# dschleef/schroedinger

Hardware: AMD Instinct MI355X
Metric: Mpix/s IIWT+OBMC decode, 2160p s16 (higher is better)
Workload: dtype s16

## Files before the change

### include/schro_hip.h

```cpp
#ifndef SCHRO_HIP_H
#define SCHRO_HIP_H

#include <stddef.h>
#include <stdint.h>

#ifdef __cplusplus
extern "C" {
#endif

#define SCHRO_HIP_OK 0
#define SCHRO_HIP_EINVAL (-1)
#define SCHRO_HIP_EDEVICE (-2)
#define SCHRO_HIP_ENOMEM (-3)
#define SCHRO_HIP_EUNSUPPORTED (-4)
#define SCHRO_HIP_ESKIPPED (-5)
#define SCHRO_HIP_ENEEDS_RESIDUAL (-6)

#define SCHRO_EXEC_DOMAIN_HIP 0x0004
#define SCHRO_MEMORY_DOMAIN_HIP 0x0008

#define SCHRO_HIP_FORMAT_DEPTH(f) ((f) & 0xc)
#define SCHRO_HIP_FORMAT_DEPTH_U8 0x00
#define SCHRO_HIP_FORMAT_DEPTH_S16 0x04
#define SCHRO_HIP_FORMAT_DEPTH_S32 0x08
// ... 19 lines not shown
int schro_hip_upload_2d (SchroHipContext * ctx, void *dst, int dst_stride,
    const void *src, int src_stride, int row_bytes, int height);
int schro_hip_download_2d (SchroHipContext * ctx, void *dst, int dst_stride,
    const void *src, int src_stride, int row_bytes, int height);
int schro_hip_memset (SchroHipContext * ctx, void *dst, int value,
    size_t bytes);
void *schro_hip_host_alloc (size_t size);
void schro_hip_host_free (void *ptr);
int schro_hip_upload_2d_async (SchroHipContext * ctx, void *dst, int dst_stride,
    const void *src, int src_stride, int row_bytes, int height);
int schro_hip_download_2d_async (SchroHipContext * ctx, void *dst, int dst_stride,
    const void *src, int src_stride, int row_bytes, int height);
int schro_hip_queue_synchronize (SchroHipContext * ctx, int queue);
int schro_hip_queue_set_cu_mask (SchroHipContext * ctx, int queue, const uint32_t * mask, int words);
int schro_hip_synchronize (SchroHipContext * ctx);
void *schro_hip_stream (SchroHipContext * ctx);

#define SCHRO_HIP_QUEUES 4
#define SCHRO_HIP_QUEUE_H2D 2
#define SCHRO_HIP_QUEUE_D2H 3
int schro_hip_context_select_queue (SchroHipContext * ctx, int queue);
int schro_hip_context_queue (SchroHipContext * ctx);
int schro_hip_queue_wait (SchroHipContext * ctx, int waiter, int signaller);
#define SCHRO_HIP_MARKS 16
int schro_hip_queue_mark (SchroHipContext * ctx, int mark);
int schro_hip_queue_wait_mark (SchroHipContext * ctx, int mark);
int schro_hip_queue_mark_synchronize (SchroHipContext * ctx, int mark);

int schro_hip_timer_begin (SchroHipContext * ctx);
float schro_hip_timer_end (SchroHipContext * ctx);

#define SCHRO_HIP_KERNEL_IIWT_FINEST 0
#define SCHRO_HIP_KERNEL_IIWT_COARSE 1
#define SCHRO_HIP_KERNEL_UPSAMPLE 2
#define SCHRO_HIP_KERNEL_OBMC 3
#define SCHRO_HIP_KERNEL_CONVERT 4
#define SCHRO_HIP_KERNEL_SLICES 5
#define SCHRO_HIP_KERNEL_DC_PREDICT 6
#define SCHRO_HIP_KERNEL_DEQUANT 7
#define SCHRO_HIP_KERNEL_QUANTISE 8
#define SCHRO_HIP_KERNEL_QUANTISE_DC 9
#define SCHRO_HIP_KERNEL_CLASSES 10
int schro_hip_profile_enable (SchroHipContext * ctx, int enable);
int schro_hip_profile_reset (SchroHipContext * ctx);
int schro_hip_profile_read (SchroHipContext * ctx, int kernel_class,
    double *total_ms, int *launches);

#define SCHRO_HIP_OBMC_ROUTE_ROW 0
#define SCHRO_HIP_OBMC_ROUTE_ITEM 1
#define SCHRO_HIP_OBMC_ROUTE_GENERAL 2
#define SCHRO_HIP_OBMC_ROUTE_STRIP 3
#define SCHRO_HIP_OBMC_ROUTES 4
int schro_hip_obmc_routes (SchroHipContext * ctx, long long counts[SCHRO_HIP_OBMC_ROUTES], int reset);

#define SCHRO_HIP_V210_ROUTE_HAAR3 0
#define SCHRO_HIP_V210_ROUTE_LEVEL 1
#define SCHRO_HIP_V210_ROUTE_TWO_PASS 2
#define SCHRO_HIP_V210_ROUTES 3
int schro_hip_v210_routes (SchroHipContext * ctx, long long counts[SCHRO_HIP_V210_ROUTES], int reset);

#define SCHRO_HIP_PACK8_ROUTE_LEVEL 0
#define SCHRO_HIP_PACK8_ROUTE_TWO_PASS 1
#define SCHRO_HIP_PACK8_ROUTES 2
int schro_hip_pack8_routes (SchroHipContext * ctx, long long counts[SCHRO_HIP_PACK8_ROUTES], int reset);

#define SCHRO_HIP_WIDE_ROUTE_LEVEL 0
#define SCHRO_HIP_WIDE_ROUTE_TWO_PASS 1
#define SCHRO_HIP_WIDE_ROUTES 2
int schro_hip_wide_routes (SchroHipContext * ctx, long long counts[SCHRO_HIP_WIDE_ROUTES], int reset);


typedef struct {
  const void *src;
  int src_stride;
  void *dst;
  int dst_stride;
  int width;
  int height;
  const uint8_t *pred;
  int pred_stride;
  int out_width, out_height;
  int combine;
  const void *ll;
  int ll_stride;
  int reserved;
} SchroHipIwtPlane;

int schro_hip_iiwt_batch (SchroHipContext * ctx,
    const SchroHipIwtPlane * planes, int nplanes, int depth, int filter,
    int bpp);

typedef struct {
  const void *src;
  int src_stride;
  void *dst;
  int dst_stride;
  int width;
  int height;
} SchroHipIwtFwdPlane;

int schro_hip_iwt_batch (SchroHipContext * ctx, const SchroHipIwtFwdPlane * planes, int nplanes, int depth, int filter,
    int bytes_per_sample);

typedef struct {
  const uint8_t *src;
  int src_stride;
// ... 905 lines not shown
```

### schroedinger_amd/_lib.py

```python
import ctypes as C
import os

_HERE = os.path.dirname(os.path.abspath(__file__))
LIB_PATH = os.environ.get("SCHRO_HIP_LIB") or os.path.join(_HERE, "libschro_hip.so")

EXPORTED_SYMBOLS = [
    "schro_hip_context_new", "schro_hip_context_free", "schro_hip_device_count",
    "schro_hip_last_error", "schro_hip_set_abort_on_error", "schro_hip_init", "schro_hip_thread_bind", "schro_hip_thread_bound", "schro_hip_context_set_stage_completion", "schro_hip_dequant_plan_new", "schro_hip_dequant_plan_run", "schro_hip_dequant_plan_free", "schro_hip_queue_mark_synchronize",
    "schro_hip_host_alloc", "schro_hip_host_free", "schro_hip_upload_2d_async", "schro_hip_download_2d_async",
    "schro_hip_queue_synchronize", "schro_hip_queue_set_cu_mask", "schro_memory_domain_new_hip_host", "schro_hip_codeblock_layout",
    "schro_frame_to_hip_async", "schro_hipframe_to_cpu_async", "schro_hip_frame_copy_to",
    "schro_upsampled_hipframe_upsample_inplace",
    "schro_hip_scheduler_new_on", "schro_hip_scheduler_publish_reference", "schro_hip_scheduler_reference_frame",
    "schro_hip_scheduler_moves", "schro_hip_scheduler_skipped", "schro_hip_scheduler_refs_in_flight_max",
    "schro_hip_domain_alloc", "schro_hip_domain_free", "schro_hip_domain_bytes",
    "schro_hip_upload_2d", "schro_hip_download_2d", "schro_hip_memset",
    "schro_hip_synchronize", "schro_hip_stream",
    "schro_memory_domain_new_hip", "schro_memory_domain_free_hip", "schro_hip_domain_context",
    "schro_hip_context_domain",
    "schro_hip_obmc_stamps_dump",
    "schro_hip_scheduler_new", "schro_hip_scheduler_new_virtual", "schro_hip_scheduler_free",
    "schro_hip_scheduler_n_devices", "schro_hip_scheduler_context", "schro_hip_scheduler_submit",
    "schro_hip_scheduler_retire", "schro_hip_scheduler_wait",
    "schro_hip_context_select_queue", "schro_hip_context_queue", "schro_hip_queue_wait",
    "schro_hip_queue_mark", "schro_hip_queue_wait_mark",
    "schro_hip_timer_begin", "schro_hip_timer_end",
    "schro_hip_profile_enable", "schro_hip_profile_reset", "schro_hip_profile_read", "schro_hip_obmc_routes",
    "schro_hip_v210_routes", "schro_hip_pack8_routes", "schro_hip_wide_routes",
    "schro_hip_iiwt_batch", "schro_hip_iwt_batch", "schro_hipframe_iwt_transform", "schro_hip_convert_u8_batch", "schro_hip_upsample_batch",
    "schro_hip_downsample_batch", "schro_hip_metric_scan_setup", "schro_hip_metric_scan_batch", "schro_hipframe_downsample",
    "schro_rough_me_heirarchical_scan_nohint_hip",
    "schro_hip_rough_hint_batch", "schro_hip_rough_me_batch", "schro_hip_rough_hint_check", "schro_hip_rough_me_check",
    "schro_rough_me_heirarchical_scan_hint_hip", "schro_rough_me_heirarchical_scan_hip",
    "schro_hip_hbm_level_batch", "schro_hip_hbm_batch", "schro_hip_hbm_level_check", "schro_hip_hbm_check",
    "schro_hierarchical_bm_scan_hint_hip", "schro_hbm_scan_hip",
    "schro_hip_subpel_error_batch", "schro_hip_subpel_choose_batch", "schro_hip_subpel_batch", "schro_hip_subpel_check",
    "schro_encoder_motion_predict_subpel_deep_hip",
    "schro_hip_split2_metric_batch", "schro_hip_split2_choose_batch", "schro_hip_split2_batch", "schro_hip_split2_check",
    "schro_mode_decision_split2_hip",
    "schro_hip_mode_metric_batch", "schro_hip_mode_choose_batch", "schro_hip_mode_decision_batch", "schro_hip_mode_decision_check",
    "schro_mode_decision_hip",
    "schro_hip_upsampled_bytes", "schro_hip_upsampled_download", "schro_hip_upsampled_pair_bytes",
    "schro_hip_upsampled_pair_download", "schro_hip_pack_u8_batch",
    "schro_hip_pack_v210_batch", "schro_hip_iiwt_pack_v210_batch", "schro_hip_iiwt_pack_u8_batch", "schro_hip_pack_wide_batch", "schro_hip_shift_right_batch",
    "schro_hip_iiwt_pack_wide_batch",
    "schro_hipframe_shift_right", "schro_hip_add_batch", "schro_hipframe_add",
    "schro_hip_lowdelay_arith", "schro_hip_lowdelay_batch", "schro_hip_dc_predict_batch",
    "schro_hip_lowdelay_encode_batch", "schro_hip_encode_lowdelay_transform_data",
    "schro_hip_noarith_encode_bound", "schro_hip_noarith_encode_batch", "schro_hip_noarith_encode_check",
    "schro_hip_encode_transform_data_noarith",
    "schro_hip_noarith_decode_batch", "schro_hip_noarith_decode_check", "schro_hip_noarith_decode_scratch_words",
    "schro_hipframe_decode_transform_data_noarith",
    "schro_hip_motion_encode_bound", "schro_hip_motion_encode_batch", "schro_hip_motion_encode_check",
    "schro_hip_encode_motion_data_noarith",
    "schro_hip_motion_decode_batch", "schro_hip_motion_decode_check", "schro_hip_motion_decode_scratch_words",
    "schro_hip_decode_motion_data_noarith",
    "schro_hip_dequant_batch", "schro_hip_quantise_batch", "schro_hip_subtract_batch", "schro_hipframe_subtract",
    "schro_hipframe_quantise", "schro_hip_histogram_batch", "schro_hipframe_subband_histograms",
    "schro_hip_decode_lowdelay_transform_data", "schro_hipframe_dequantise",
    "schro_hip_obmc_batch", "schro_hip_obmc_prediction_epoch", "schro_hip_obmc_overflowed",
    "schro_hip_frame_new_and_alloc", "schro_hip_frame_ref", "schro_hip_frame_unref",
    "schro_frame_to_hip", "schro_hipframe_to_cpu",
    "schro_frame_inverse_iwt_transform_hip", "schro_frame_inverse_iwt_transform_combine_hip", "schro_frame_inverse_iwt_transform_convert_hip",
    "schro_frame_inverse_iwt_transform_combine_convert_hip", "schro_frame_inverse_iwt_transform_shift_convert_hip",
    "schro_upsampled_hipframe_upsample",
    "schro_motion_render_hip", "schro_hipframe_convert",
]


class IwtPlane(C.Structure):
    _fields_ = [("src", C.c_void_p), ("src_stride", C.c_int),
                ("dst", C.c_void_p), ("dst_stride", C.c_int),
                ("width", C.c_int), ("height", C.c_int),
                ("pred", C.c_void_p), ("pred_stride", C.c_int),
                ("out_width", C.c_int), ("out_height", C.c_int), ("combine", C.c_int),
                ("ll", C.c_void_p), ("ll_stride", C.c_int), ("reserved", C.c_int)]


class IwtFwdPlane(C.Structure):
    _fields_ = [("src", C.c_void_p), ("src_stride", C.c_int),
# ... 414 lines not shown
    L.schro_hip_frame_copy_to.restype = vp
    L.schro_upsampled_hipframe_upsample_inplace.argtypes = [vp]
    L.schro_upsampled_hipframe_upsample_inplace.restype = i
    L.schro_hip_scheduler_new_on.argtypes = [C.POINTER(C.c_int), i]
    L.schro_hip_scheduler_new_on.restype = vp
    L.schro_hip_scheduler_publish_reference.argtypes = [vp, i, vp]
    L.schro_hip_scheduler_publish_reference.restype = i
    L.schro_hip_scheduler_reference_frame.argtypes = [vp, i, i]
    L.schro_hip_scheduler_reference_frame.restype = vp
    L.schro_hip_scheduler_moves.argtypes = [vp]
    L.schro_hip_scheduler_moves.restype = C.c_long
    L.schro_hip_scheduler_skipped.argtypes = [vp]
    L.schro_hip_scheduler_skipped.restype = C.c_long
    L.schro_hip_scheduler_refs_in_flight_max.argtypes = [vp]
    L.schro_hip_scheduler_refs_in_flight_max.restype = i
    L.schro_hip_scheduler_new.argtypes = [i]
    L.schro_hip_scheduler_new.restype = vp
    L.schro_hip_scheduler_new_virtual.argtypes = [i]
    L.schro_hip_scheduler_new_virtual.restype = vp
    L.schro_hip_scheduler_free.argtypes = [vp]
    L.schro_hip_scheduler_free.restype = None
    L.schro_hip_scheduler_n_devices.argtypes = [vp]
    L.schro_hip_scheduler_n_devices.restype = i
    L.schro_hip_scheduler_context.argtypes = [vp, i]
    L.schro_hip_scheduler_context.restype = vp
    L.schro_hip_scheduler_submit.argtypes = [vp, i, C.POINTER(C.c_int), i, i, PICTURE_FUNC, vp, C.POINTER(C.c_int)]
    L.schro_hip_scheduler_submit.restype = i
    L.schro_hip_scheduler_retire.argtypes = [vp, i]
    L.schro_hip_scheduler_retire.restype = i
    L.schro_hip_scheduler_wait.argtypes = [vp]
    L.schro_hip_scheduler_wait.restype = i
    L.schro_hip_context_select_queue.argtypes = [vp, i]
    L.schro_hip_context_select_queue.restype = i
    L.schro_hip_context_queue.argtypes = [vp]
    L.schro_hip_context_queue.restype = i
    L.schro_hip_queue_wait.argtypes = [vp, i, i]
    L.schro_hip_queue_wait.restype = i
    L.schro_hip_queue_mark.argtypes = [vp, i]
    L.schro_hip_queue_mark.restype = i
    L.schro_hip_queue_wait_mark.argtypes = [vp, i]
    L.schro_hip_queue_wait_mark.restype = i
    L.schro_hip_timer_begin.argtypes = [vp]
    L.schro_hip_timer_begin.restype = i
    L.schro_hip_timer_end.argtypes = [vp]
    L.schro_hip_timer_end.restype = C.c_float
    L.schro_hip_profile_enable.argtypes = [vp, i]
    L.schro_hip_profile_enable.restype = i
    L.schro_hip_profile_reset.argtypes = [vp]
    L.schro_hip_profile_reset.restype = i
    L.schro_hip_profile_read.argtypes = [vp, i, C.POINTER(C.c_double), C.POINTER(C.c_int)]
    L.schro_hip_profile_read.restype = i
    L.schro_hip_obmc_routes.argtypes = [vp, C.POINTER(C.c_longlong), i]
    L.schro_hip_obmc_routes.restype = i
    L.schro_hip_v210_routes.argtypes = [vp, C.POINTER(C.c_longlong), i]
    L.schro_hip_v210_routes.restype = i
    L.schro_hip_pack8_routes.argtypes = [vp, C.POINTER(C.c_longlong), i]
    L.schro_hip_pack8_routes.restype = i
    L.schro_hip_wide_routes.argtypes = [vp, C.POINTER(C.c_longlong), i]
    L.schro_hip_wide_routes.restype = i
    L.schro_hip_iiwt_batch.argtypes = [vp, C.POINTER(IwtPlane), i, i, i, i]
    L.schro_hip_iiwt_batch.restype = i
    L.schro_hip_iwt_batch.argtypes = [vp, C.POINTER(IwtFwdPlane), i, i, i, i]
    L.schro_hip_iwt_batch.restype = i
    L.schro_hipframe_iwt_transform.argtypes = [vp, C.POINTER(Frame), C.POINTER(Params)]
    L.schro_hipframe_iwt_transform.restype = i
    L.schro_hip_downsample_batch.argtypes = [vp, C.POINTER(DownsamplePlane), i]
    L.schro_hip_downsample_batch.restype = i
    L.schro_hip_metric_scan_setup.argtypes = [C.POINTER(MetricScan), i, i, i, i, i, i]
    L.schro_hip_metric_scan_setup.restype = i
    L.schro_hip_metric_scan_batch.argtypes = [vp, C.POINTER(MetricScanPicture), i]
    L.schro_hip_metric_scan_batch.restype = i
    L.schro_hipframe_downsample.argtypes = [C.POINTER(Frame), C.POINTER(Frame)]
    L.schro_hipframe_downsample.restype = i
    L.schro_rough_me_heirarchical_scan_nohint_hip.argtypes = [C.POINTER(Frame), C.POINTER(Frame), C.POINTER(Params), i, i, i, vp]
    L.schro_rough_me_heirarchical_scan_nohint_hip.restype = i
    L.schro_hip_rough_hint_batch.argtypes = [vp, C.POINTER(RoughHintPicture), i]
    L.schro_hip_rough_hint_batch.restype = i
    L.schro_hip_rough_me_batch.argtypes = [vp, C.POINTER(RoughChain), i, i, i]
    L.schro_hip_rough_me_batch.restype = i
    L.schro_hip_rough_hint_check.argtypes = [C.POINTER(RoughHintPicture), i]
    L.schro_hip_rough_hint_check.restype = i
    L.schro_hip_rough_me_check.argtypes = [C.POINTER(RoughChain), i, i, i]
    L.schro_hip_rough_me_check.restype = i
    L.schro_rough_me_heirarchical_scan_hint_hip.argtypes = [C.POINTER(Frame), C.POINTER(Frame), C.POINTER(Params), i, i, i, vp, vp]
    L.schro_rough_me_heirarchical_scan_hint_hip.restype = i
    L.schro_rough_me_heirarchical_scan_hip.argtypes = [C.POINTER(C.POINTER(Frame)), C.POINTER(C.POINTER(Frame)), C.POINTER(Params), i, i,
                                                       C.POINTER(vp)]
    L.schro_rough_me_heirarchical_scan_hip.restype = i
    L.schro_hip_hbm_level_batch.argtypes = [vp, C.POINTER(HbmLevel), i]
    L.schro_hip_hbm_level_batch.restype = i
    L.schro_hip_hbm_batch.argtypes = [vp, C.POINTER(HbmChain), i, i]
    L.schro_hip_hbm_batch.restype = i
    L.schro_hip_hbm_level_check.argtypes = [C.POINTER(HbmLevel), i]
    L.schro_hip_hbm_level_check.restype = i
    L.schro_hip_hbm_check.argtypes = [C.POINTER(HbmChain), i, i]
    L.schro_hip_hbm_check.restype = i
    L.schro_hierarchical_bm_scan_hint_hip.argtypes = [C.POINTER(Frame), C.POINTER(Frame), C.POINTER(Params), i, i, i, vp, vp]
    L.schro_hierarchical_bm_scan_hint_hip.restype = i
    L.schro_hbm_scan_hip.argtypes = [C.POINTER(C.POINTER(Frame)), C.POINTER(C.POINTER(Frame)), C.POINTER(Params), i, i, i,
                                     C.POINTER(C.c_void_p)]
    L.schro_hbm_scan_hip.restype = i
    L.schro_hip_subpel_error_batch.argtypes = [vp, C.POINTER(SubpelChain), i, i, C.POINTER(C.c_void_p)]
    L.schro_hip_subpel_error_batch.restype = i
    L.schro_hip_subpel_choose_batch.argtypes = [vp, C.POINTER(SubpelChain), i, i, C.POINTER(C.c_void_p)]
    L.schro_hip_subpel_choose_batch.restype = i
    L.schro_hip_subpel_batch.argtypes = [vp, C.POINTER(SubpelChain), i]
# ... 179 lines not shown
```

### schroedinger_amd/csrc/obmc_row.hip

```cpp

#include "obmc_row_body.h"

namespace schro {
namespace {

SCHRO_ROW_KERNEL (obmc_row_kernel_2_1, 6, 2, 1)
SCHRO_ROW_KERNEL (obmc_row_kernel_2_2, 6, 2, 2)
SCHRO_ROW_KERNEL (obmc_row_kernel_3_1, 7, 3, 1)
SCHRO_ROW_KERNEL (obmc_row_kernel_3_2, 5, 3, 2)
SCHRO_ROW_KERNEL (obmc_row_kernel_4_1, 6, 4, 1)
SCHRO_ROW_KERNEL (obmc_row_kernel_4_2, 5, 4, 2)
SCHRO_ROW_KERNEL (obmc_row_kernel_uv_2, 5, 2, 1, true)
SCHRO_ROW_KERNEL (obmc_row_kernel_uv_3, 7, 3, 1, true)
SCHRO_ROW_KERNEL (obmc_row_kernel_uv_4, 6, 4, 1, true)
SCHRO_ROW_KERNEL (obmc_row_kernel_p_2_1, 6, 2, 1, false, kRTH, true)
SCHRO_ROW_KERNEL (obmc_row_kernel_p_3_1, 8, 3, 1, false, kRTH, true)
#ifdef SCHRO_HIP_EXPERIMENTS
SCHRO_ROW_KERNEL (obmc_row_kernel_p_3_1_pad, 8, 3, 1, false, kRTH, true, 1, 1, false, true)
#endif
SCHRO_ROW_KERNEL (obmc_row_kernel_p_4_1, 7, 4, 1, false, kRTH, true)
SCHRO_ROW_KERNEL (obmc_row_kernel_p_uv_2, 5, 2, 1, true, kRTH, true)
SCHRO_ROW_KERNEL (obmc_row_kernel_p_uv_3, 8, 3, 1, true, kRTH, true)
SCHRO_ROW_KERNEL (obmc_row_kernel_p_uv_4, 7, 4, 1, true, kRTH, true)
SCHRO_ROW_KERNEL (obmc_row_kernel_h2_3_1, 6, 3, 1, false, kRTH, false, 1, 2)
// ... 184 lines not shown
    uint32_t v = 0;
    if (r < j.yblen && u >= 0) {
      if (uv)
        v = (uint32_t) (wx[u] * wy[r]) * 0x00010001u;
      else
        v = (uint32_t) (wx[2 * u] * wy[r]) | ((uint32_t) (wx[2 * u + 1] * wy[r]) << 16);
    }
    out[i] = v;
  }
  for (int t = 0; t < 4 * xf; t++) {
    const int type = t / xf, pr = t - type * xf;
    const int u = ns == 1 ? pr : unit_of (pr);
    out[wcap + t] = u < 0 ? 0u : uv ? (uint32_t) folded (wx, u, j.xblen, j.xbsep, j.xoff, type) * 0x00010001u
        : (uint32_t) folded (wx, 2 * u, j.xblen, j.xbsep, j.xoff, type) | ((uint32_t) folded (wx, 2 * u + 1, j.xblen, j.xbsep, j.xoff, type) << 16);
  }
  const int fy = wcap + 4 * xf;
  for (int t = 0; t < 128; t++)
    out[fy + t] = (uint32_t) folded (wy, t & 31, j.yblen, j.ybsep, j.yoff, t >> 5);
  for (int i = 0; i < wxn; i++)
    out[fy + 128 + i] = (uint32_t) wx[i];
  for (int i = 0; i < 32; i++)
    out[fy + 128 + wxn + i] = (uint32_t) wy[i];
}

void
obmc_row_tile_record (const ObmcJob & j, bool uv, int ns, int tx, int ty, uint32_t * rec)
{
  const int tw = obmc_row_tile_width (uv);
  const int x_lo = tx * tw, y_lo = ty * kRTH, x_hi = std::min (x_lo + tw, j.w), y_hi = std::min (y_lo + kRTH, j.h);
  const int i_lo = std::max (0, (x_lo + j.xoff - j.xblen + 2 * j.xbsep) / j.xbsep - 1);
  const int i_hi = std::min (j.nbx - 1, (x_hi - 1 + j.xoff) / j.xbsep);
  const int j_lo = std::max (0, (y_lo + j.yoff - j.yblen + 2 * j.ybsep) / j.ybsep - 1);
  const int j_hi = std::min (j.nby - 1, (y_hi - 1 + j.yoff) / j.ybsep);
  const int nbi = std::max (0, std::min (255, (i_hi - i_lo + 1) * ns)), nbj = std::max (0, std::min (255, j_hi - j_lo + 1));
  const uint32_t m16 = nbi > 1 ? (65536u + (uint32_t) nbi - 1u) / (uint32_t) nbi : 0u;
  rec[0] = (uint32_t) x_lo | ((uint32_t) y_lo << 16);
  rec[1] = (uint32_t) i_lo | ((uint32_t) j_lo << 16);
  rec[2] = (uint32_t) nbi | ((uint32_t) nbj << 8) | (m16 << 16);
}

int
obmc_row_tile_height ()
{
  return kRTH;
}

int
obmc_row_tile_width (bool uv)
{
  return row_caps (3, 1, uv).tw;
}

}
```

### schroedinger_amd/csrc/obmc_row_body.h

```cpp

#pragma once

#include "schro_hip_internal.h"
#include "obmc_common.h"
#include <algorithm>
#include <cstdlib>

namespace schro {
namespace {

constexpr int kRThreads = 256;
constexpr int kRTH = 32;
template < int ND, bool UV, int NS = 1 > struct RowGeo {
  static constexpr int kTW = UV ? 64 : 128;
  static constexpr int kMargin = UV ? (ND <= 3 && NS == 1 ? 5 : 8) : (ND <= 2 ? 8 : 16);
  static constexpr int kAccW = UV ? (ND <= 3 && NS == 1 ? 75 : 81) : (ND <= 2 ? 73 : 85);
  static constexpr int kBlk = ND <= 2 ? 344 : (NS > 1 ? (UV ? 208 : 144) : UV ? (ND == 3 ? 180 : 192) : 128) * kRTH / 32,
      kItem = ND <= 2 ? 1792 : (NS > 1 ? 1664 : UV ? (ND == 3 ? 960 : 1152) : (ND == 3 ? 1024 : 1152)) * kRTH / 32;
  static constexpr int kWRow = 2 * ND * NS;
  static constexpr int kWCap = 32 * kWRow;
  static constexpr int kXF = NS == 1 ? 8 : kWRow, kWxN = NS == 1 ? 16 : 32;
  static constexpr bool kPadBlk = UV || ND > 2;
  static constexpr int kWFoldY = kWCap + 4 * kXF, kWRampX = kWFoldY + 128, kWRampY = kWRampX + kWxN;
  static constexpr int kWTab = kWRampY + 32;
};
constexpr int kRBoth = 0, kRRef0 = 1, kRRef1 = 2, kRDc = 3, kREdge = 4, kRRim = 5;
constexpr int kRSlots = 16 + 4 + 4 + 3;
__host__ __device__ constexpr int
row_slot_base (int cls)
{
  return cls == kRBoth ? 0 : cls == kRRef0 ? 16 : cls == kRRef1 ? 20 : cls == kRDc ? 24 : cls == kREdge ? 25 : 26;
}

typedef unsigned short u16x2 __attribute__ ((ext_vector_type (2)));
typedef short s16x2 __attribute__ ((ext_vector_type (2)));

struct __attribute__ ((aligned (4))) RowRef {
  int base;
  uint32_t ydb;
  int dci;
};

template < bool PAD > struct alignas (PAD ? 4 : 8) RowBlkT {
  int16_t y, x;
  uint32_t fr;
  RowRef r[2];
  uint32_t pad[PAD ? 1 : 0];
};
static_assert (sizeof (RowBlkT < true >) == 36 && sizeof (RowBlkT < false >) == 32, "block records: an odd number of words / r03's");

template < typename B >
__device__ __forceinline__ uint32_t
blk_flags (const B & hb)
{
  return hb.fr >> 16;
}

template < typename B >
__device__ __forceinline__ uint32_t
blk_ry (const B & hb, int r)
{
  return (hb.fr >> (16 + 6 + r)) & 1u;
}

template < typename B >
__device__ __forceinline__ int
blk_dc (const B & hb, int pl)
{
  return pl ? hb.r[0].base >> 16 : (int) (int16_t) hb.r[0].base;
}


struct __attribute__ ((aligned (8))) PlaneIO {
  const uint8_t *ref[2];
  const void *residual;
  uint8_t *out;
  int residual_stride, out_stride;
};

__device__ __forceinline__ uint32_t
lerp1 (uint32_t a, uint32_t b)
{
  return __builtin_amdgcn_lerp (a, b, 0x01010101u);
}
// ... 39 lines not shown
__device__ __forceinline__ void
issue_run (__amdgpu_buffer_rsrc_t ref, uint32_t off, RawRun < ND > &r)
{
  const uint32_t al = off & ~3u;
  r.sh = off & 3u;
  if constexpr (ND == 1) {
    const u32x2 q = __builtin_amdgcn_raw_buffer_load_b64 (ref, (int) al, 0, kGatherAux);
    r.c[0] = q.x;
    r.c[1] = q.y;
  } else if constexpr (ND == 2) {
    typedef uint32_t u32x3 __attribute__ ((ext_vector_type (3)));
    const u32x3 q = __builtin_amdgcn_raw_buffer_load_b96 (ref, (int) al, 0, kGatherAux);
    r.c[0] = q.x;
    r.c[1] = q.y;
    r.c[2] = q.z;
  } else if constexpr (ND == 3) {
    const u32x4 q = __builtin_amdgcn_raw_buffer_load_b128 (ref, (int) al, 0, kGatherAux);
    r.c[0] = q.x;
    r.c[1] = q.y;
    r.c[2] = q.z;
    r.c[3] = q.w;
  } else {
    const u32x4 q = __builtin_amdgcn_raw_buffer_load_b128 (ref, (int) al, 0, kGatherAux);
    const u32x2 q2 = __builtin_amdgcn_raw_buffer_load_b64 (ref, (int) al + 16, 0, kGatherAux);
    r.c[0] = q.x;
    r.c[1] = q.y;
    r.c[2] = q.z;
    r.c[3] = q.w;
    r.c[4] = q2.x;
  }
}

template < int ND >
__device__ __forceinline__ void
align_run (const RawRun < ND > &r, uint32_t * d)
{
#pragma unroll
  for (int k = 0; k < ND; k++)
    d[k] = __builtin_amdgcn_alignbyte (r.c[k + 1], r.c[k], r.sh);
}

__device__ __forceinline__ uint32_t
row_ofs (uint32_t y, uint32_t stride)
{
  return __umul24 (y >> 2, stride) + ((y & 3u) << 5);
}

template < int ND, bool ABS = false, bool W = false >
__device__ __forceinline__ void
predict_row (const ObmcJob & job, __amdgpu_buffer_rsrc_t ref, uint32_t stride, const RowRef & rr, uint32_t ry, int row, uint32_t * out)
{
  const int dB = (int) rr.ydb >> 16;
  uint32_t offA, offC = 0;
  bool any_b, any_c;
  if constexpr (ABS) {
    const int hy = (int) (int16_t) (rr.ydb & 0xffffu) + 2 * row, gh = 2 * job.h - 2;
    const uint32_t Y0 = (uint32_t) clampi (hy, 0, gh), Y1 = (uint32_t) clampi (hy + (int) ry, 0, gh);
    offA = (uint32_t) rr.base + ((Y0 & 1u) << 8) + row_ofs (Y0 >> 1, stride);
    offC = (uint32_t) rr.base + ((Y1 & 1u) << 8) + row_ofs (Y1 >> 1, stride);
    any_b = any_c = true;
  } else {
    const uint32_t y = (rr.ydb & 0xffffu) + (uint32_t) row;
    offA = (uint32_t) rr.base + row_ofs (y, stride);
    any_b = __ballot (dB != 0) != 0;
    any_c = __ballot ((W ? rr.dci & ~0xf0 : rr.dci) != 0) != 0;
    if (any_c)
      offC = (uint32_t) (rr.base + (rr.dci >> 16)) + row_ofs (y + ((uint32_t) rr.dci & 1u), stride);
  }
  RawRun < ND > qa, qb, qc, qd;
  issue_run < ND > (ref, offA, qa);
  if (any_b)
    issue_run < ND > (ref, offA + (uint32_t) dB, qb);
  if (any_c) {
    issue_run < ND > (ref, offC, qc);
    if (any_b)
      issue_run < ND > (ref, offC + (uint32_t) dB, qd);
  }
  uint32_t a[ND];
  align_run < ND > (qa, a);
  if constexpr (W) {
    const uint32_t rx = ((uint32_t) rr.dci >> 4) & 3u, rw = ((uint32_t) rr.dci >> 6) & 3u;
    const uint32_t w00 = (4u - rw) * (4u - rx), w01 = (4u - rw) * rx, w10 = rw * (4u - rx), w11 = rw * rx;
    uint32_t lo[ND], hi[ND];
#pragma unroll
    for (int k = 0; k < ND; k++) {
      lo[k] = __umul24 (__builtin_amdgcn_perm (0u, a[k], 0x0c010c00u), w00) + 0x00080008u;
      hi[k] = __umul24 (__builtin_amdgcn_perm (0u, a[k], 0x0c030c02u), w00) + 0x00080008u;
    }
    auto add_tap = [&] (const RawRun < ND > &q, uint32_t w) {
      uint32_t t[ND];
      align_run < ND > (q, t);
#pragma unroll
      for (int k = 0; k < ND; k++) {
        lo[k] += __umul24 (__builtin_amdgcn_perm (0u, t[k], 0x0c010c00u), w);
        hi[k] += __umul24 (__builtin_amdgcn_perm (0u, t[k], 0x0c030c02u), w);
      }
    };
    if (any_b)
      add_tap (qb, w01);
    if (any_c) {
      add_tap (qc, w10);
      if (any_b)
        add_tap (qd, w11);
    }
#pragma unroll
    for (int k = 0; k < ND; k++)
      out[k] = __builtin_amdgcn_perm (hi[k] >> 4, lo[k] >> 4, 0x06040200u);
    return;
  }
  if (!any_c) {
    if (!any_b) {
#pragma unroll
      for (int k = 0; k < ND; k++)
        out[k] = a[k];
    } else {
      uint32_t b[ND];
      align_run < ND > (qb, b);
#pragma unroll
      for (int k = 0; k < ND; k++)
        out[k] = lerp1 (a[k], b[k]);
    }
  } else if (!any_b) {
    uint32_t c[ND];
    align_run < ND > (qc, c);
#pragma unroll
    for (int k = 0; k < ND; k++)
      out[k] = lerp1 (a[k], c[k]);
  } else {
    uint32_t b[ND], c[ND], d[ND];
    align_run < ND > (qb, b);
    align_run < ND > (qc, c);
    align_run < ND > (qd, d);
#pragma unroll
    for (int k = 0; k < ND; k++) {
      const uint32_t h0 = lerp1 (a[k], b[k]), h1 = lerp1 (c[k], d[k]);
      out[k] = __builtin_amdgcn_lerp (h0, h1, ~((a[k] ^ b[k]) | (c[k] ^ d[k])));
    }
  }
}

template < int ND > struct TapRuns {
  RawRun < ND > qa, qb, qc, qd;
  bool any_b, any_c;
};

template < int ND >
__device__ __forceinline__ void
issue_taps (__amdgpu_buffer_rsrc_t ref, uint32_t stride, const RowRef & rr, int row, TapRuns < ND > &t)
{
  const int dB = (int) rr.ydb >> 16;
  const uint32_t y = (rr.ydb & 0xffffu) + (uint32_t) row;
  const uint32_t offA = (uint32_t) rr.base + row_ofs (y, stride);
  t.any_b = __ballot (dB != 0) != 0;
  t.any_c = __ballot (rr.dci != 0) != 0;
  issue_run < ND > (ref, offA, t.qa);
  if (t.any_b)
    issue_run < ND > (ref, offA + (uint32_t) dB, t.qb);
  if (t.any_c) {
    const uint32_t offC = (uint32_t) (rr.base + (rr.dci >> 16)) + row_ofs (y + ((uint32_t) rr.dci & 1u), stride);
    issue_run < ND > (ref, offC, t.qc);
    if (t.any_b)
      issue_run < ND > (ref, offC + (uint32_t) dB, t.qd);
  }
}

template < int ND >
__device__ __forceinline__ void
finish_taps (const TapRuns < ND > &t, uint32_t * out)
{
  uint32_t a[ND];
  align_run < ND > (t.qa, a);
  if (!t.any_c) {
    if (!t.any_b) {
#pragma unroll
      for (int k = 0; k < ND; k++)
        out[k] = a[k];
    } else {
      uint32_t b[ND];
      align_run < ND > (t.qb, b);
#pragma unroll
// ... 81 lines not shown
      issue_run < NH > (ref_b, off, qv);
      align_run < NH > (qu, u);
      align_run < NH > (qv, v);
    }
    interleave_uv < ND > (u, v, out);
  } else if constexpr (RK == 0) {
    if constexpr (ABS)
      predict_row_plain_abs < ND > (job, ref, stride, rr, row, out);
    else
      predict_row_plain < ND > (ref, stride, rr, row, out);
  } else if constexpr (RK == 3) {
    predict_row < ND, ABS, true > (job, ref, stride, rr, ABS ? (((uint32_t) rr.dci & 0xc0u) ? 1u : 0u) : 0u, row, out);
  } else {
    predict_row < ND, ABS > (job, ref, stride, rr, ry, row, out);
  }
}

__device__ __forceinline__ uint32_t
blend_weighted (uint32_t a, uint32_t b, uint32_t w1, uint32_t w2, uint32_t round2, uint32_t bits)
{
  const uint32_t lo = __umul24 (__builtin_amdgcn_perm (0u, a, 0x0c010c00u), w1) + __umul24 (__builtin_amdgcn_perm (0u, b, 0x0c010c00u), w2) + round2;
  const uint32_t hi = __umul24 (__builtin_amdgcn_perm (0u, a, 0x0c030c02u), w1) + __umul24 (__builtin_amdgcn_perm (0u, b, 0x0c030c02u), w2) + round2;
  return __builtin_amdgcn_perm (hi >> bits, lo >> bits, 0x06040200u);
}

struct RowRefs {
  __amdgpu_buffer_rsrc_t rsrc[2];
  uint32_t stride[2];
  __amdgpu_buffer_rsrc_t rsrc_b[2];
};

template < bool UV, typename B >
__device__ __forceinline__ uint32_t
dc_bytes (const B & hb, int pl)
{
  if constexpr (UV)
    return ((uint32_t) (blk_dc (hb, 0) & 0xff) | ((uint32_t) (blk_dc (hb, 1) & 0xff) << 8)) * 0x00010001u;
  else
    return (uint32_t) (blk_dc (hb, pl) & 0xff) * 0x01010101u;
}

template < int ND, bool UV, int CLS, bool EXACT, int RK, int NS, bool WP, bool PAD = false >
__device__ __forceinline__ void
row_pass (const ObmcJob & job, int pl, const RowRefs & refs, const uint16_t * s_item, const RowBlkT < RowGeo < ND, UV, NS >::kPadBlk > *s_hot,
    const uint32_t * s_wp, uint32_t * acc, int par, int it, int hi)
{
  typedef RowGeo < ND, UV, NS > G;
  const int e = s_item[min (it, hi - 1)];
  const auto & hb = s_hot[e & 0x1ff];
  const int row = PAD ? (e >> 9) & 63 : e >> 9;
  constexpr bool weighted = WP;
  const uint32_t wround = WP ? (uint32_t) ((1 << job.wbits) >> 1) * 0x00010001u : 0u;
  uint32_t p[ND];
  if constexpr (CLS == kRDc) {
#pragma unroll
    for (int k = 0; k < ND; k++)
      p[k] = dc_bytes < UV > (hb, pl);
  } else if constexpr (CLS == kREdge) {
    uint32_t p1[ND];
    predict < ND, RK, true, UV > (job, refs.rsrc[0], refs.rsrc_b[0], refs.stride[0], hb.r[0], blk_ry (hb, 0), row, p);
    __builtin_amdgcn_sched_barrier (0);
    predict < ND, RK, true, UV > (job, refs.rsrc[1], refs.rsrc_b[1], refs.stride[1], hb.r[1], blk_ry (hb, 1), row, p1);
    const uint32_t mode = blk_flags (hb) & 3u;
    const uint32_t dc = dc_bytes < UV > (hb, pl);
    const uint32_t m0 = (mode & 1u) ? 0xffffffffu : 0u, m1 = (mode & 2u) ? 0xffffffffu : 0u;
#pragma unroll
    for (int k = 0; k < ND; k++) {
      const uint32_t a = (p[k] & m0) | (p1[k] & ~m0), b = (p1[k] & m1) | (p[k] & ~m1);
      p[k] = mode ? (weighted ? blend_weighted (a, b, (uint32_t) job.w1, (uint32_t) job.w2, wround, (uint32_t) job.wbits) : lerp1 (a, b)) : dc;
    }
  } else if constexpr (CLS == kRBoth) {
    uint32_t p1[ND];
#if defined (SCHRO_HIP_EXPERIMENTS) && defined (SCHRO_ROW_BOTH_AT_ONCE)
    if constexpr (RK == 1) {
      TapRuns < ND > t0, t1;
      issue_taps < ND > (refs.rsrc[0], refs.stride[0], hb.r[0], row, t0);
      issue_taps < ND > (refs.rsrc[1], refs.stride[1], hb.r[1], row, t1);
      __builtin_amdgcn_sched_barrier (0);
      finish_taps < ND > (t0, p);
      finish_taps < ND > (t1, p1);
    } else
#endif
    {
    predict < ND, RK, false, UV > (job, refs.rsrc[0], refs.rsrc_b[0], refs.stride[0], hb.r[0], 0u, row, p);
    __builtin_amdgcn_sched_barrier (0);
    predict < ND, RK, false, UV > (job, refs.rsrc[1], refs.rsrc_b[1], refs.stride[1], hb.r[1], 0u, row, p1);
    }
    if (weighted) {
#pragma unroll
      for (int k = 0; k < ND; k++)
        p[k] = blend_weighted (p[k], p1[k], (uint32_t) job.w1, (uint32_t) job.w2, wround, (uint32_t) job.wbits);
    } else {
#pragma unroll
      for (int k = 0; k < ND; k++)
        p[k] = lerp1 (p[k], p1[k]);
    }
  } else {
    constexpr int r = CLS == kRRef1 ? 1 : 0;
    predict < ND, RK, false, UV > (job, refs.rsrc[r], refs.rsrc_b[r], refs.stride[r], hb.r[r], 0u, row, p);
  }
  if (it >= hi || (PAD && (e & 0x8000)))
    return;
#if defined (SCHRO_HIP_EXPERIMENTS) && defined (SCHRO_ROW_PASS_LOADS_ONLY)
  {
    uint32_t x = 0;
#pragma unroll
// ... 522 lines not shown
        flags = gload < uint32_t > (mvp);
        v01 = gload < uint32_t > (mvp + 12);
        v23 = gload < uint32_t > (mvp + 16);
      }
      const int bx = xbsep * i - xoff, by = ybsep * jj - yoff;
      RowBlk info;
      info.x = (int16_t) (bx + seg * seglen - x_lo);
      info.y = (int16_t) (by - y_lo);
      const int mode = flags & 3;
      const bool interior = i >= 1 && i < job.max_x_blocks && jj >= 1 && jj < job.max_y_blocks;
      auto dc_of = [&] (int comp) {
        const int dc = comp == 0 ? (int16_t) (v01 & 0xffff) : comp == 1 ? (int16_t) (v01 >> 16) : (int16_t) (v23 & 0xffff);
        return interior ? (int) (int16_t) (dc + 128) : (int) (uint8_t) (dc + 128);
      };
      const int pdc = dc_of (job.comp), pdc_b = (nplanes > 1 || UV) ? dc_of (job.comp_b) : 0;
      const int dcs = (int) (((uint32_t) pdc & 0xffffu) | ((uint32_t) pdc_b << 16));
      uint32_t bflags = (uint32_t) mode | ((uint32_t) seg << 8);
      int taps[2] = { 0, 0 };
      RowRef in_ref[2], edge_ref[2];
      bool off_h = false, clamped_v = false;
#pragma unroll
      for (int r = 0; r < 2; r++) {
        int fx, fy;
        mv_origin (job, bx, by, v01, v23, r, &fx, &fy);
        fx += (seg * seglen) * (1 << prec);
        const bool used = (mode & (r + 1)) != 0;
        if constexpr (RK == 0) {
          const bool in_h = fx >= 0 && fx + seglen <= job.w, in_v = fy >= 0 && fy + yblen <= job.h;
          clamped_v |= used && !(in_h && in_v);
          in_ref[r].base = used && in_h && in_v ? fx : 0;
          in_ref[r].ydb = used && in_h && in_v ? (uint32_t) fy : 0u;
          in_ref[r].dci = 0;
          edge_ref[r].base = used ? fx : 0;
          edge_ref[r].ydb = used ? (uint32_t) fy & 0xffffu : 0u;
          edge_ref[r].dci = 0;
        } else {
          const int hx = RK == 3 ? fx >> 2 : prec >= 2 ? fx >> 1 : fx, hy = RK == 3 ? fy >> 2 : prec >= 2 ? fy >> 1 : fy;
          const int rx = RK == 3 ? fx & 3 : prec >= 2 ? fx & 1 : 0, ry = RK == 3 ? fy & 3 : prec >= 2 ? fy & 1 : 0;
          const int wbits = RK == 3 ? (rx << 4) | (ry << 6) : 0;
          const int xp = ((hx >> 1) + kHpApron) << ps, px = hx & 1, py = hy & 1;
          const bool in_h = xp >= 0 && (xp >> 4) < (job.ref_stride[r] >> 9) && (unsigned) (hy + 16384) < 32768u;
          const bool in_v = hy >= 0 && hy + 2 * (yblen - 1) + 1 <= gh;
          off_h |= used && !in_h;
          clamped_v |= used && !in_v;
          const int colbase = in_h && used ? (xp >> 4) * 512 + (xp & 15) + px * 128 : 0;
          const uint32_t dB = in_h && used && rx ? (uint32_t) (px ? (1 << ps) - 128 : 128) : 0u;
          in_ref[r].base = colbase + (in_h && used ? py * 256 : 0);
          in_ref[r].ydb = (in_h && in_v && used ? (uint32_t) (hy >> 1) : 0u) | (dB << 16);
          in_ref[r].dci = in_h && used ? ((ry ? (py ? (int) (((uint32_t) -256 << 16) | 1u) : (int) (256u << 16)) : 0) | wbits) : 0;
          edge_ref[r].base = colbase;
          edge_ref[r].ydb = (in_h && used ? (uint32_t) hy & 0xffffu : 0u) | (dB << 16);
          edge_ref[r].dci = in_h && used ? wbits : 0;
          bflags |= (uint32_t) (in_h && used && ry ? 1 : 0) << (6 + r);
          taps[r] = in_h && used ? (rx ? 1 : 0) | (ry ? 2 : 0) : 0;
        }
      }
      info.r[0] = in_ref[0];
      info.r[1] = in_ref[1];
      const int ra = max (0, -(int) info.y), rb = min (yblen, y_hi - by);
      int fold = (by < yoff ? 1 : 0) | (by + yblen > yfold_hi ? 2 : 0) | (bx < xoff ? 4 : 0) | (bx + xblen > xfold_hi ? 8 : 0);
      if (NS > 1)
        fold &= seg == 0 ? ~8 : ~4;
      const bool wide_dc = mode == 0 && ((unsigned) pdc > 255u || (unsigned) pdc_b > 255u);
      if (wide_dc) {
        s_wide = 1;
        if (overflow)
          __hip_atomic_store (overflow, 1u, __ATOMIC_RELAXED, __HIP_MEMORY_SCOPE_SYSTEM);
      }
      int key, nrows = rb - ra;
      if (off_h || wide_dc || yblen > 32 || xblen > NS * (UV ? 8 : 16)) {
        key = kRRim;
        if (seg == 0) {
          int fx, fy;
          mv_origin (job, bx, by, v01, v23, 0, &fx, &fy);
          info.r[0].base = (int) (((uint32_t) fx & 0xffffu) | ((uint32_t) fy << 16));
          mv_origin (job, bx, by, v01, v23, 1, &fx, &fy);
          info.r[1].base = (int) (((uint32_t) fx & 0xffffu) | ((uint32_t) fy << 16));
          s_rim[atomicAdd (&s_nrim, 1)] = (uint16_t) blk;
        }
      } else if (fold || clamped_v) {
        key = kREdge;
        info.r[0] = edge_ref[0];
        info.r[1] = edge_ref[1];
        bflags |= (uint32_t) fold << 2;
      } else if (mode == 3) {
        key = kRBoth;
      } else if (mode == 0) {
        key = kRDc;
      } else {
        key = mode == 1 ? kRRef0 : kRRef1;
      }
      if (NS > 1 && ((int) info.x + seglen <= 0 || (int) info.x >= kRTW))
        nrows = 0;
      int nitems = nrows;
      if constexpr (PAD) {
        if ((key == kRBoth || key == kRRef0 || key == kRRef1) && nrows > 0) {
          const uint32_t y_first = (info.r[key == kRRef1 ? 1 : 0].ydb & 0xffffu) + (uint32_t) ra;
          const int front = (int) (y_first & 3u), padded = (front + nrows + 3) & ~3, pad = padded - nrows;
          if (pad && atomicSub (&s_padleft, pad) < pad) {
            key = kREdge;
            info.r[0] = edge_ref[0];
            info.r[1] = edge_ref[1];
          } else {
            bflags |= (uint32_t) front << 9;
            nitems = padded;
          }
        }
      }
      const int slot = row_slot_base (key) + (key == kRBoth ? taps[0] | (taps[1] << 2) : key == kRRef0 ? taps[0] : key == kRRef1 ? taps[1] : 0);
      if (mode == 0)
        info.r[0].base = dcs;
      info.fr = (uint32_t) ra | ((uint32_t) nrows << 8) | (bflags << 16);
      s_hot[blk] = info;
      const int istart = key == kRRim ? 0 : atomicAdd (&s_icnt[slot], nitems);
      s_meta[blk] = (uint16_t) (slot | (istart << 5));
    }
  }
  __syncthreads ();
  RSTAMP (2);
  int sbase;
  {
    const int lane = tid & 63;
    const int cnt = lane < kRSlots ? s_icnt[lane] : 0;
    static_assert (kRSlots <= 32, "the scan covers two rows of 16 lanes");
    int incl = cnt;
    incl += __builtin_amdgcn_update_dpp (0, incl, 0x111, 0xf, 0xf, true);
    incl += __builtin_amdgcn_update_dpp (0, incl, 0x112, 0xf, 0xf, true);
    incl += __builtin_amdgcn_update_dpp (0, incl, 0x114, 0xf, 0xf, true);
    incl += __builtin_amdgcn_update_dpp (0, incl, 0x118, 0xf, 0xf, true);
    incl += __builtin_amdgcn_update_dpp (0, incl, 0x142, 0xa, 0xf, false);
    sbase = incl - cnt;
  }
#pragma unroll
  for (int c = 0; c <= kRRim; c++)
    ibase[c] = __builtin_amdgcn_readlane (sbase, row_slot_base (c));
  for (int b0 = 0; b0 < nblk; b0 += kRThreads) {
    const int blk = b0 + tid;
    const bool have = blk < nblk;
    const int meta = have ? s_meta[blk] : 0, slot = meta & 31;
    const int ib = __shfl (sbase, slot);
    if (!have || slot == row_slot_base (kRRim))
      continue;
    const int rows = (int) s_hot[blk].fr, ra = rows & 0xff, n = (rows >> 8) & 0xff;
    uint16_t *ip = s_item + ib + (meta >> 5);
    typedef uint32_t u32_a2 __attribute__ ((aligned (2), may_alias));
    typedef u32x2 u32x2_a2 __attribute__ ((aligned (2), may_alias));
    if constexpr (PAD) {
      if (slot < row_slot_base (kRDc) && n > 0) {
        const int front = (rows >> 25) & 3, total = (front + n + 3) & ~3;
#pragma clang loop vectorize(disable) unroll(disable)
        for (int j = 0; j < total; j += 4) {
          uint32_t it4[4];
#pragma unroll
          for (int q = 0; q < 4; q++) {
            const int idx = j + q - front;
            it4[q] = (uint32_t) (blk | ((ra + min (max (idx, 0), n - 1)) << 9)) | ((unsigned) idx >= (unsigned) n ? 0x8000u : 0u);
          }
          *reinterpret_cast < u32x2_a2 * >(ip + j) = (u32x2) { it4[0] | (it4[1] << 16), it4[2] | (it4[3] << 16) };
        }
        continue;
      }
    }
// ... 26 lines not shown
    io.residual_stride = pl ? job.residual_stride_b : job.residual_stride;
    io.out_stride = pl ? job.out_stride_b : job.out_stride;
    PlaneIO iov = io;
    if constexpr (UV) {
      if constexpr (RK == 0) {
        iov.ref[0] = job.ref_b[0];
        iov.ref[1] = job.ref_b[1];
      }
      iov.residual = job.residual_b;
      iov.out = job.out_b;
      iov.residual_stride = job.residual_stride_b;
      iov.out_stride = job.out_stride_b;
    }
    constexpr bool kEarlyRes = ND >= 3 && NP == 1 && !NORES;
    const bool s16 = !NORES && job.out_s16;
    const bool fast = s16 ? row_finish_s16_is_fast < G > (io, x_lo, x_hi) && (!UV || row_finish_s16_is_fast < G > (iov, x_lo, x_hi))
        : row_finish_is_fast < G > (job, io, x_lo, x_hi) && (!UV || row_finish_is_fast < G > (job, iov, x_lo, x_hi));
    constexpr int kRounds = kRFinishRounds < TH, G >;
    u32x4 res[UV ? 2 * kRounds : kRounds];
#define SCHRO_ROW_PREFETCH() do { \
      if constexpr (UV) { \
        row_finish_prefetch < TH, G, 2, 0 > (io, tid, x_lo, y_lo, y_hi, res); \
        row_finish_prefetch < TH, G, 2, 1 > (iov, tid, x_lo, y_lo, y_hi, res); \
      } else { \
        row_finish_prefetch < TH, G, 1, 0 > (io, tid, x_lo, y_lo, y_hi, res); \
      } } while (0)
    if constexpr (kEarlyRes) {
      if (fast)
        SCHRO_ROW_PREFETCH ();
      __builtin_amdgcn_sched_barrier (0);
    }
    int turn = 0;
    RowRefs refs;
#pragma unroll
    for (int r = 0; r < 2; r++) {
      refs.stride[r] = (uint32_t) job.ref_stride[r];
      const uint32_t bytes = RK == 0 ? (uint32_t) job.ref_stride[r] * (uint32_t) (job.h - 1) + (((uint32_t) job.w + 3u) & ~3u)
          : (uint32_t) job.ref_stride[r] * (uint32_t) ((job.h + 3) >> 2);
      refs.rsrc[r] = __builtin_amdgcn_make_buffer_rsrc ((void *) io.ref[r], 0, (int) bytes, 0x00020000);
      refs.rsrc_b[r] = refs.rsrc[r];
      if constexpr (UV && RK == 0)
        refs.rsrc_b[r] = __builtin_amdgcn_make_buffer_rsrc ((void *) iov.ref[r], 0, (int) bytes, 0x00020000);
    }
#define SCHRO_ROW_CLASS(C) row_class < ND, UV, C, RK, NS, WP, PAD > (job, pl, refs, s_item, s_hot, s_wp, acc, par, \
    ibase[C], ibase[C + 1], exact, &turn)
#pragma unroll
    for (int rep_ = 0; rep_ < kRepPasses; rep_++) {
      SCHRO_ROW_CLASS (kRBoth);
      SCHRO_ROW_CLASS (kRRef0);
      SCHRO_ROW_CLASS (kRRef1);
      SCHRO_ROW_CLASS (kRDc);
      SCHRO_ROW_CLASS (kREdge);
    }
#undef SCHRO_ROW_CLASS
    RSTAMP (4);
    if (nrim > 0) {
      const int nseg = (xblen + 3) >> 2, per_block = yblen * nseg;
      const uint32_t m_per_block = div_magic (per_block), m_nseg = div_magic (nseg);
      for (int item = tid; item < nrim * per_block; item += kRThreads) {
        const int b = mdiv (item, per_block, m_per_block);
        const int rem = item - b * per_block;
        const int r2 = mdiv (rem, nseg, m_nseg), s2 = rem - r2 * nseg;
        const RowBlk & hb = s_hot[s_rim[b]];
        const int bx = hb.x + x_lo, by = hb.y + y_lo;
        const int y = by + r2, xs = bx + 4 * s2;
        if (y < y_lo || y >= y_hi || xs + 3 < x_lo || xs >= x_hi)
          continue;
        const int fx[2] = { (int) (int16_t) hb.r[0].base, (int) (int16_t) hb.r[1].base }, fy[2] = { hb.r[0].base >> 16, hb.r[1].base >> 16 };
#define SCHRO_ROW_SLOW(cb, dcpl) do { \
          const int md = (int) (blk_flags (hb) & 3u) | (blk_dc (hb, dcpl) << 8);        \
          if constexpr (RK == 0) \
            row_slow < 0, G, UV > (job, (UV && cb) ? iov : io, cb, bx, by, md, fx, fy, r2, s2, x_lo, y_lo, xfold_hi, yfold_hi, s_wx, s_wy, acc, par, exact); \
          else if (RK == 1 && job.prec == 1) \
            row_slow < 1, G, UV > (job, io, cb, bx, by, md, fx, fy, r2, s2, x_lo, y_lo, xfold_hi, yfold_hi, s_wx, s_wy, acc, par, exact); \
          else \
            row_slow < 2, G, UV > (job, io, cb, bx, by, md, fx, fy, r2, s2, x_lo, y_lo, xfold_hi, yfold_hi, s_wx, s_wy, acc, par, exact); \
        } while (0)
        if constexpr (UV) {
          SCHRO_ROW_SLOW (0, 0);
          SCHRO_ROW_SLOW (1, 1);
        } else {
          SCHRO_ROW_SLOW (0, pl);
        }
#undef SCHRO_ROW_SLOW
      }
    }
    RSTAMP (5);
    if constexpr (NORES) {
#pragma unroll
      for (int n = 0; n < (UV ? 2 * kRounds : kRounds); n++)
        res[n] = (u32x4) { 0u, 0u, 0u, 0u };
    } else if constexpr (!kEarlyRes) {
      if (fast)
        SCHRO_ROW_PREFETCH ();
    }
#undef SCHRO_ROW_PREFETCH
    __syncthreads ();
    RSTAMP (6);
#pragma unroll
    for (int rep_ = 0; rep_ < kRepFinish; rep_++)
    if (s16) {
      if constexpr (UV) {
        if (fast) {
          row_finish_s16_uv < TH, G > (io, iov, acc, tid, x_lo, y_lo, y_hi);
        } else {
          row_finish_s16_plain < TH, G, true > (io, 0, acc, par, tid, x_lo, y_lo, x_hi, y_hi);
// ... 97 lines not shown
```

Measured before the change: 204,600.

## Merge OBMC row tap classes by tap count and fold 2-tap blends

Row items in the OBMC kernel are now bucketed by how many taps each reference needs (1, 2 or 4) rather than by the exact horizontal/vertical combination, which cuts the slot count from 27 to 18. Horizontal-only and vertical-only 2-tap cases now share one code path that issues a single extra load and blends it with one lerp. The aim is fewer specialised class passes and less wave divergence, so each sorted bucket is fuller. It also adds a host query for the slot mapping and an experiment-only empty-pass hook that is off by default.

```diff
diff --git a/include/schro_hip.h b/include/schro_hip.h
--- a/include/schro_hip.h
+++ b/include/schro_hip.h
@@ -95,6 +95,9 @@
 #define SCHRO_HIP_OBMC_ROUTE_STRIP 3
 #define SCHRO_HIP_OBMC_ROUTES 4
 int schro_hip_obmc_routes (SchroHipContext * ctx, long long counts[SCHRO_HIP_OBMC_ROUTES], int reset);
+
+#define SCHRO_HIP_OBMC_ROW_SLOTS 18
+int schro_hip_obmc_row_slot (int item_class, int taps_1, int taps_2);
 
 #define SCHRO_HIP_V210_ROUTE_HAAR3 0
 #define SCHRO_HIP_V210_ROUTE_LEVEL 1
diff --git a/schroedinger_amd/_lib.py b/schroedinger_amd/_lib.py
--- a/schroedinger_amd/_lib.py
+++ b/schroedinger_amd/_lib.py
@@ -26,6 +26,7 @@
     "schro_hip_queue_mark", "schro_hip_queue_wait_mark",
     "schro_hip_timer_begin", "schro_hip_timer_end",
     "schro_hip_profile_enable", "schro_hip_profile_reset", "schro_hip_profile_read", "schro_hip_obmc_routes",
+    "schro_hip_obmc_row_slot",
     "schro_hip_v210_routes", "schro_hip_pack8_routes", "schro_hip_wide_routes",
     "schro_hip_iiwt_batch", "schro_hip_iwt_batch", "schro_hipframe_iwt_transform", "schro_hip_convert_u8_batch", "schro_hip_upsample_batch",
     "schro_hip_downsample_batch", "schro_hip_metric_scan_setup", "schro_hip_metric_scan_batch", "schro_hipframe_downsample",
@@ -546,6 +547,8 @@
     L.schro_hip_profile_read.restype = i
     L.schro_hip_obmc_routes.argtypes = [vp, C.POINTER(C.c_longlong), i]
     L.schro_hip_obmc_routes.restype = i
+    L.schro_hip_obmc_row_slot.argtypes = [i, i, i]
+    L.schro_hip_obmc_row_slot.restype = i
     L.schro_hip_v210_routes.argtypes = [vp, C.POINTER(C.c_longlong), i]
     L.schro_hip_v210_routes.restype = i
     L.schro_hip_pack8_routes.argtypes = [vp, C.POINTER(C.c_longlong), i]
diff --git a/schroedinger_amd/csrc/obmc_row.hip b/schroedinger_amd/csrc/obmc_row.hip
--- a/schroedinger_amd/csrc/obmc_row.hip
+++ b/schroedinger_amd/csrc/obmc_row.hip
@@ -260,3 +260,20 @@
 }
 
 }
+
+extern "C" {
+
+int
+schro_hip_obmc_row_slot (int item_class, int taps_1, int taps_2)
+{
+  using namespace schro;
+  static_assert (kRSlots == SCHRO_HIP_OBMC_ROW_SLOTS && row_slot (kRRim, 0, 0) == kRSlots - 1, "include/schro_hip.h: the slots");
+  auto taps_ok = [](int n) { return n == 1 || n == 2 || n == 4; };
+  if (item_class < kRBoth || item_class > kRRim)
+    return -1;
+  if (((item_class == kRBoth || item_class == kRRef0) && !taps_ok (taps_1)) || ((item_class == kRBoth || item_class == kRRef1) && !taps_ok (taps_2)))
+    return -1;
+  return row_slot (item_class, taps_1, taps_2);
+}
+
+}
diff --git a/schroedinger_amd/csrc/obmc_row_body.h b/schroedinger_amd/csrc/obmc_row_body.h
--- a/schroedinger_amd/csrc/obmc_row_body.h
+++ b/schroedinger_amd/csrc/obmc_row_body.h
@@ -25,11 +25,19 @@
   static constexpr int kWTab = kWRampY + 32;
 };
 constexpr int kRBoth = 0, kRRef0 = 1, kRRef1 = 2, kRDc = 3, kREdge = 4, kRRim = 5;
-constexpr int kRSlots = 16 + 4 + 4 + 3;
+constexpr int kRNone = 6;
+constexpr int kRSlots = 9 + 3 + 3 + 3;
 __host__ __device__ constexpr int
 row_slot_base (int cls)
 {
-  return cls == kRBoth ? 0 : cls == kRRef0 ? 16 : cls == kRRef1 ? 20 : cls == kRDc ? 24 : cls == kREdge ? 25 : 26;
+  return cls == kRBoth ? 0 : cls == kRRef0 ? 9 : cls == kRRef1 ? 12 : cls == kRDc ? 15 : cls == kREdge ? 16 : 17;
+}
+
+__host__ __device__ constexpr int
+row_slot (int cls, int n0, int n1)
+{
+  const int c0 = n0 >= 4 ? 2 : n0 >= 2 ? 1 : 0, c1 = n1 >= 4 ? 2 : n1 >= 2 ? 1 : 0;
+  return row_slot_base (cls) + (cls == kRBoth ? (int) ((0x210457368ull >> (4 * (c0 + 3 * c1))) & 15u) : cls == kRRef0 ? c0 : cls == kRRef1 ? c1 : 0);
 }
 
 typedef unsigned short u16x2 __attribute__ ((ext_vector_type (2)));
@@ -175,29 +183,30 @@
 {
   const int dB = (int) rr.ydb >> 16;
   uint32_t offA, offC = 0;
-  bool any_b, any_c;
+  bool any4, any2;
   if constexpr (ABS) {
     const int hy = (int) (int16_t) (rr.ydb & 0xffffu) + 2 * row, gh = 2 * job.h - 2;
     const uint32_t Y0 = (uint32_t) clampi (hy, 0, gh), Y1 = (uint32_t) clampi (hy + (int) ry, 0, gh);
     offA = (uint32_t) rr.base + ((Y0 & 1u) << 8) + row_ofs (Y0 >> 1, stride);
     offC = (uint32_t) rr.base + ((Y1 & 1u) << 8) + row_ofs (Y1 >> 1, stride);
-    any_b = any_c = true;
+    any4 = any2 = true;
   } else {
     const uint32_t y = (rr.ydb & 0xffffu) + (uint32_t) row;
     offA = (uint32_t) rr.base + row_ofs (y, stride);
-    any_b = __ballot (dB != 0) != 0;
-    any_c = __ballot ((W ? rr.dci & ~0xf0 : rr.dci) != 0) != 0;
-    if (any_c)
+    const bool lane_b = dB != 0, lane_c = (W ? rr.dci & ~0xf0 : rr.dci) != 0;
+    any4 = __ballot (lane_b && lane_c) != 0;
+    any2 = any4 || __ballot (lane_b || lane_c) != 0;
+    if (any2)
       offC = (uint32_t) (rr.base + (rr.dci >> 16)) + row_ofs (y + ((uint32_t) rr.dci & 1u), stride);
   }
   RawRun < ND > qa, qb, qc, qd;
   issue_run < ND > (ref, offA, qa);
-  if (any_b)
+  if (any4) {
     issue_run < ND > (ref, offA + (uint32_t) dB, qb);
-  if (any_c) {
     issue_run < ND > (ref, offC, qc);
-    if (any_b)
-      issue_run < ND > (ref, offC + (uint32_t) dB, qd);
+    issue_run < ND > (ref, offC + (uint32_t) dB, qd);
+  } else if (any2) {
+    issue_run < ND > (ref, offC + (uint32_t) dB, qb);
   }
   uint32_t a[ND];
   align_run < ND > (qa, a);
@@ -219,36 +228,28 @@
         hi[k] += __umul24 (__builtin_amdgcn_perm (0u, t[k], 0x0c030c02u), w);
       }
     };
-    if (any_b)
+    if (any4) {
       add_tap (qb, w01);
-    if (any_c) {
       add_tap (qc, w10);
-      if (any_b)
-        add_tap (qd, w11);
+      add_tap (qd, w11);
+    } else if (any2) {
+      add_tap (qb, w01 + w10);
     }
 #pragma unroll
     for (int k = 0; k < ND; k++)
       out[k] = __builtin_amdgcn_perm (hi[k] >> 4, lo[k] >> 4, 0x06040200u);
     return;
   }
-  if (!any_c) {
-    if (!any_b) {
-#pragma unroll
-      for (int k = 0; k < ND; k++)
-        out[k] = a[k];
-    } else {
-      uint32_t b[ND];
-      align_run < ND > (qb, b);
-#pragma unroll
-      for (int k = 0; k < ND; k++)
-        out[k] = lerp1 (a[k], b[k]);
-    }
-  } else if (!any_b) {
-    uint32_t c[ND];
-    align_run < ND > (qc, c);
+  if (!any2) {
 #pragma unroll
     for (int k = 0; k < ND; k++)
-      out[k] = lerp1 (a[k], c[k]);
+      out[k] = a[k];
+  } else if (!any4) {
+    uint32_t b[ND];
+    align_run < ND > (qb, b);
+#pragma unroll
+    for (int k = 0; k < ND; k++)
+      out[k] = lerp1 (a[k], b[k]);
   } else {
     uint32_t b[ND], c[ND], d[ND];
     align_run < ND > (qb, b);
@@ -436,6 +437,15 @@
   constexpr bool weighted = WP;
   const uint32_t wround = WP ? (uint32_t) ((1 << job.wbits) >> 1) * 0x00010001u : 0u;
   uint32_t p[ND];
+#if defined (SCHRO_HIP_EXPERIMENTS) && defined (SCHRO_ROW_EMPTY_PASSES)
+  if constexpr (CLS == kRNone) {
+#pragma unroll
+    for (int k = 0; k < ND; k++) {
+      p[k] = 0u;
+      asm volatile ("" : "+v" (p[k]));
+    }
+  } else
+#endif
   if constexpr (CLS == kRDc) {
 #pragma unroll
     for (int k = 0; k < ND; k++)
@@ -1064,7 +1074,7 @@
           edge_ref[r].ydb = (in_h && used ? (uint32_t) hy & 0xffffu : 0u) | (dB << 16);
           edge_ref[r].dci = in_h && used ? wbits : 0;
           bflags |= (uint32_t) (in_h && used && ry ? 1 : 0) << (6 + r);
-          taps[r] = in_h && used ? (rx ? 1 : 0) | (ry ? 2 : 0) : 0;
+          taps[r] = in_h && used ? 1 << ((rx ? 1 : 0) + (ry ? 1 : 0)) : 0;
         }
       }
       info.r[0] = in_ref[0];
@@ -1119,7 +1129,7 @@
           }
         }
       }
-      const int slot = row_slot_base (key) + (key == kRBoth ? taps[0] | (taps[1] << 2) : key == kRRef0 ? taps[0] : key == kRRef1 ? taps[1] : 0);
+      const int slot = row_slot (key, taps[0], taps[1]);
       if (mode == 0)
         info.r[0].base = dcs;
       info.fr = (uint32_t) ra | ((uint32_t) nrows << 8) | (bflags << 16);
@@ -1252,6 +1262,10 @@
       SCHRO_ROW_CLASS (kRDc);
       SCHRO_ROW_CLASS (kREdge);
     }
+#if defined (SCHRO_HIP_EXPERIMENTS) && defined (SCHRO_ROW_EMPTY_PASSES)
+    for (int n = 0; n < SCHRO_ROW_EMPTY_PASSES; n++)
+      row_class < ND, UV, kRNone, RK, NS, WP, PAD > (job, pl, refs, s_item, s_hot, s_wp, acc, par, 0, min (64, ibase[kREdge]), exact, &turn);
+#endif
 #undef SCHRO_ROW_CLASS
     RSTAMP (4);
     if (nrim > 0) {
```

New measurement: 207,300, median of 4. About the same (+1.3%).
